# alibaba/TorchEasyRec

Measured on NVIDIA B200. Metric: samples/sec (DLRM-Criteo synth, train step fwd+bwd+optimizer), higher is better.
Workload: dtype f32

## Files before the change

### torcheasyrec_b200/csrc/tzk_gemm3x.cu

```cuda
#include <stdint.h>
#include <stdio.h>
#include <stdlib.h>

#include "tzk_umma_desc.h"
#ifdef TZK_CPU_SHIM
#include "cuda_cpu_shim.h"
#include "tcgen05_cpu_emu.h"
#else
#include <cuda.h>
#include <cuda_runtime.h>
#define TZK_DYN_SMEM(type, name) extern __shared__ __align__(1024) type name[]
#define TZK_UNPAREN(...) __VA_ARGS__
#define TZK_LAUNCH(kernel, grid, block, smem, stream, ...) TZK_UNPAREN kernel<<<grid, block, smem, stream>>>(__VA_ARGS__)
#endif

namespace {
#ifndef TZK_CPU_SHIM
#include "tzk_tcgen05_ptx.h"
#endif

constexpr int BK = 32;
constexpr int UK = 8;
constexpr int X_BYTES = BM * BK * 4;
constexpr int NUM_THREADS = 192;
template <int BN>
struct Cfg {
  static constexpr int W_BYTES = BN * BK * 4;
  static constexpr int W_PAD = (W_BYTES + 1023) / 1024 * 1024;
  static constexpr int STAGE_BYTES = 2 * X_BYTES + 2 * W_PAD;
  static constexpr int P = BN <= 64 ? 3 : 1;
  static constexpr int P_STACKED = BN <= 64 ? 2 : 1;
  static constexpr int TMEM_COLS = 512;
  static constexpr int STAGES = BN <= 64 ? 4 : 3;
};

__device__ __forceinline__ float tf32_trunc(float x) { return __uint_as_float(__float_as_uint(x) & 0xffffe000u); }

struct Params {
  const float* bias;
  float* y;
  int64_t ld_y;
  int64_t M;
  int K;
  int N;
  int relu;
};

constexpr int PF_DIST = 12;
template <int BN, bool STACK, int TW, bool RAW, bool SPLIT, bool PF>
__global__ void __launch_bounds__(64 + 32 * TW + (SPLIT ? 128 : 0), 1)
gemm3x_kernel(const __grid_constant__ CUtensorMap map_x, const __grid_constant__ CUtensorMap map_whi,
              const __grid_constant__ CUtensorMap map_wlo, Params p) {
  constexpr int W_BYTES = Cfg<BN>::W_BYTES, W_PAD = Cfg<BN>::W_PAD, STAGE_BYTES = Cfg<BN>::STAGE_BYTES;
  constexpr int TMEM_COLS = Cfg<BN>::TMEM_COLS, STAGES = Cfg<BN>::STAGES;
  constexpr int P = STACK ? Cfg<BN>::P_STACKED : Cfg<BN>::P;
  constexpr int ACC_COLS = STACK ? P * 2 * BN : (P + 1) * BN;
  static_assert(2 * ACC_COLS <= TMEM_COLS, "two tiles in flight must fit TMEM");
  static_assert(!STACK || W_PAD == W_BYTES, "stacked B needs W_hi and W_lo contiguous");
  TZK_DYN_SMEM(uint8_t, smem);
  uint8_t* stage_base = smem;
  uint64_t* bars = reinterpret_cast<uint64_t*>(smem + STAGES * STAGE_BYTES);
  uint64_t* full = bars;
  uint64_t* ready = bars + STAGES;
  uint64_t* empty = bars + 2 * STAGES;
  uint64_t* acc_full = bars + 3 * STAGES;
  uint64_t* acc_empty = bars + 3 * STAGES + 2;
  uint32_t* tmem_slot = reinterpret_cast<uint32_t*>(bars + 3 * STAGES + 4);

  const int warp = threadIdx.x >> 5, lane = threadIdx.x & 31;
  const int num_k = p.K / BK;
  const int n_used = num_k < P ? num_k : P;
  const int n_tiles = p.N / BN;
  const int64_t num_tiles = (p.M + BM - 1) / BM * n_tiles;

  if (warp == 0 && lane == 0) {
    for (int s = 0; s < STAGES; ++s) {
      mbar_init(full + s, 1);
      mbar_init(ready + s, TW);
      mbar_init(empty + s, 1);
    }
    for (int a = 0; a < 2; ++a) {
      mbar_init(acc_full + a, 1);
      mbar_init(acc_empty + a, SPLIT ? 4 : TW);
    }
    fence_mbarrier_init();
  }
  if (warp == 1) tmem_alloc(tmem_slot, TMEM_COLS);
  tc_fence_before();
  __syncthreads();
  tc_fence_after();
  const uint32_t tmem_base = *tmem_slot;

  if (warp == 0) {
    if (lane == 0) {
      int stage = 0;
      uint32_t phase = 0;
      auto load_chunk = [&](int64_t t, int kb) {
        mbar_wait(empty + stage, phase ^ 1);
        uint8_t* sb = stage_base + stage * STAGE_BYTES;
        mbar_expect_tx(full + stage, X_BYTES + 2 * W_BYTES);
        tma_load_2d(sb, &map_x, full + stage, kb * BK, (int)(t / n_tiles * BM));
        tma_load_2d(sb + 2 * X_BYTES, &map_whi, full + stage, kb * BK, (int)(t % n_tiles) * BN);
        tma_load_2d(sb + 2 * X_BYTES + W_PAD, &map_wlo, full + stage, kb * BK, (int)(t % n_tiles) * BN);
        if (++stage == STAGES) { stage = 0; phase ^= 1; }
      };
      if constexpr (PF) {
        int64_t pt = blockIdx.x;
        int pkb = 0;
        auto prefetch_next = [&] {
          if (pt < num_tiles) {
            tma_prefetch_2d(&map_x, pkb * BK, (int)(pt / n_tiles * BM));
            if (++pkb == num_k) { pkb = 0; pt += gridDim.x; }
          }
        };
        for (int i = 0; i < PF_DIST; ++i) prefetch_next();
        for (int64_t t = blockIdx.x; t < num_tiles; t += gridDim.x)
          for (int kb = 0; kb < num_k; ++kb) {
            prefetch_next();
            load_chunk(t, kb);
          }
      } else {
        for (int64_t t = blockIdx.x; t < num_tiles; t += gridDim.x)
          for (int kb = 0; kb < num_k; ++kb) load_chunk(t, kb);
      }
    }
  } else if (warp == 1) {
    int stage = 0;
    uint32_t phase = 0;
    int acc = 0;
    uint32_t acc_phase = 0;
    constexpr uint32_t idesc = make_idesc<BN>();
    constexpr uint32_t idesc2 = make_idesc<2 * BN>();
    for (int64_t t = blockIdx.x; t < num_tiles; t += gridDim.x) {
      mbar_wait_all(acc_empty + acc, acc_phase ^ 1);
      tc_fence_after();
      const uint32_t d_tmem = tmem_base + acc * ACC_COLS;
      uint32_t started = 0;
      for (int kb = 0; kb < num_k; ++kb) {
        mbar_wait_all(ready + stage, phase);
        tc_fence_after();
        if (lane == 0) {
          const uint32_t sb = smem_u32(stage_base + stage * STAGE_BYTES);
          const uint32_t a_hi = sb, a_lo = sb + X_BYTES, b_hi = sb + 2 * X_BYTES, b_lo = b_hi + W_PAD;
          const int part = kb * n_used / num_k;
#pragma unroll
          for (int k = 0; k < BK / UK; ++k) {
            const uint32_t ko = k * UK * 4;
            const uint32_t more = (started >> part) & 1u;
            if (STACK) {
              const uint32_t region = d_tmem + part * 2 * BN;
              mma_tf32(region, make_desc(a_hi + ko), make_desc(b_hi + ko), idesc2, more);
              mma_tf32(region + BN, make_desc(a_lo + ko), make_desc(b_hi + ko), idesc, 1u);
            } else {
              const uint32_t small = d_tmem + P * BN;
              mma_tf32(d_tmem + part * BN, make_desc(a_hi + ko), make_desc(b_hi + ko), idesc, more);
              mma_tf32(small, make_desc(a_lo + ko), make_desc(b_hi + ko), idesc, (started >> P) & 1u);
              mma_tf32(small, make_desc(a_hi + ko), make_desc(b_lo + ko), idesc, 1u);
            }
            started |= (1u << part) | (1u << P);
          }
          tc_commit(empty + stage);
          if (kb == num_k - 1) tc_commit(acc_full + acc);
        }
        __syncwarp();
        if (++stage == STAGES) { stage = 0; phase ^= 1; }
      }
      acc ^= 1;
      if (acc == 0) acc_phase ^= 1;
    }
  } else {
    const int tw = warp - 2;
    const int quarter = warp & 3;
    const bool do_transform = !SPLIT || tw < TW;
    const bool do_epilogue = !SPLIT || tw >= TW;
    const int part0 = SPLIT ? 0 : tw / 4, part_step = SPLIT ? 1 : TW / 4;
    int stage = 0;
    uint32_t phase = 0;
    int acc = 0;
    uint32_t acc_phase = 0;
    for (int64_t t = blockIdx.x; t < num_tiles; t += gridDim.x) {
      for (int kb = 0; do_transform && kb < num_k; ++kb) {
        mbar_wait_all(full + stage, phase);
        float4* hi = reinterpret_cast<float4*>(stage_base + stage * STAGE_BYTES);
        float4* lo = reinterpret_cast<float4*>(stage_base + stage * STAGE_BYTES + X_BYTES);
#pragma unroll
        for (int q = 0; q < X_BYTES / 16 / (TW * 32); ++q) {
          const int i = q * (TW * 32) + tw * 32 + lane;
          const float4 x = hi[i];
          float4 h, l;
          if (RAW) {
            h.x = tf32_trunc(x.x); h.y = tf32_trunc(x.y); h.z = tf32_trunc(x.z); h.w = tf32_trunc(x.w);
          } else {
            h.x = tf32_rna(x.x); h.y = tf32_rna(x.y); h.z = tf32_rna(x.z); h.w = tf32_rna(x.w);
          }
          l.x = tf32_rna(x.x - h.x); l.y = tf32_rna(x.y - h.y); l.z = tf32_rna(x.z - h.z); l.w = tf32_rna(x.w - h.w);
          if (!RAW) hi[i] = h;
          lo[i] = l;
        }
        fence_proxy_async();
        __syncwarp();
        if (lane == 0) mbar_arrive(ready + stage);
        if (++stage == STAGES) { stage = 0; phase ^= 1; }
      }
      if (!do_epilogue) continue;
      mbar_wait_all(acc_full + acc, acc_phase);
      tc_fence_after();
      const int64_t row = t / n_tiles * BM + quarter * 32 + lane;
      const int col0 = (int)(t % n_tiles) * BN;
      const uint32_t taddr = tmem_base + acc * ACC_COLS + ((uint32_t)(quarter * 32) << 16);
      float v[16];
#pragma unroll
      for (int part = part0; part < BN / 16; part += part_step) {
        float v2[16];
        if (STACK) {
          tmem_ld16(taddr + BN + part * 16, v);
          for (int q = 1; q < n_used; ++q) {
            tmem_ld16(taddr + q * 2 * BN + BN + part * 16, v2);
#pragma unroll
            for (int c = 0; c < 16; ++c) v[c] += v2[c];
          }
          for (int q = 0; q < n_used; ++q) {
            tmem_ld16(taddr + q * 2 * BN + part * 16, v2);
#pragma unroll
            for (int c = 0; c < 16; ++c) v[c] += v2[c];
          }
        } else {
          tmem_ld16(taddr + P * BN + part * 16, v);
          for (int q = 0; q < n_used; ++q) {
            tmem_ld16(taddr + q * BN + part * 16, v2);
#pragma unroll
            for (int c = 0; c < 16; ++c) v[c] += v2[c];
          }
        }
        if (row < p.M) {
          float* yr = p.y + row * p.ld_y + col0 + part * 16;
#pragma unroll
          for (int c = 0; c < 16; c += 4) {
            float4 o;
            o.x = v[c] + (p.bias ? __ldg(p.bias + col0 + part * 16 + c) : 0.f);
            o.y = v[c + 1] + (p.bias ? __ldg(p.bias + col0 + part * 16 + c + 1) : 0.f);
            o.z = v[c + 2] + (p.bias ? __ldg(p.bias + col0 + part * 16 + c + 2) : 0.f);
            o.w = v[c + 3] + (p.bias ? __ldg(p.bias + col0 + part * 16 + c + 3) : 0.f);
            if (p.relu) {
              o.x = fmaxf(o.x, 0.f); o.y = fmaxf(o.y, 0.f); o.z = fmaxf(o.z, 0.f); o.w = fmaxf(o.w, 0.f);
            }
            *reinterpret_cast<float4*>(yr + c) = o;
          }
        }
      }
      tc_fence_before();
      __syncwarp();
      if (lane == 0) mbar_arrive(acc_empty + acc);
      acc ^= 1;
      if (acc == 0) acc_phase ^= 1;
    }
  }
  tc_fence_before();
  __syncthreads();
  if (warp == 1) tmem_free(tmem_base, TMEM_COLS);
}

constexpr int WG_ROWS = 32;
constexpr int WG_BOX = WG_ROWS * 128;
constexpr int WG_A = 4 * WG_BOX, WG_B = 2 * WG_BOX;
constexpr int WG_STAGE = 2 * WG_A + 2 * WG_B;
constexpr int WG_STAGES = 4;
constexpr int WG_P = 7;

struct WgParams {
  float* partial;
  int64_t M;
  int64_t slab_rows;
  int k_tiles;
};

template <bool PF>
__global__ void __launch_bounds__(NUM_THREADS, 1)
wgrad3x_kernel(const __grid_constant__ CUtensorMap map_x, const __grid_constant__ CUtensorMap map_dz, WgParams p) {
  TZK_DYN_SMEM(uint8_t, smem);
  uint64_t* bars = reinterpret_cast<uint64_t*>(smem + WG_STAGES * WG_STAGE);
  uint64_t* full = bars;
  uint64_t* ready = bars + WG_STAGES;
  uint64_t* empty = bars + 2 * WG_STAGES;
  uint64_t* acc_full = bars + 3 * WG_STAGES;
  uint32_t* tmem_slot = reinterpret_cast<uint32_t*>(bars + 3 * WG_STAGES + 1);

  const int warp = threadIdx.x >> 5, lane = threadIdx.x & 31;
  const int jt = blockIdx.x % p.k_tiles;
  const int64_t slab = blockIdx.x / p.k_tiles;
  const int64_t row0 = slab * p.slab_rows;
  const int64_t rows = (p.M - row0 < p.slab_rows) ? p.M - row0 : p.slab_rows;
  const int num_c = (int)((rows + WG_ROWS - 1) / WG_ROWS);
  const int n_used = num_c < WG_P ? num_c : WG_P;

  if (warp == 0 && lane == 0) {
    for (int s = 0; s < WG_STAGES; ++s) {
      mbar_init(full + s, 1);
      mbar_init(ready + s, 4);
      mbar_init(empty + s, 1);
    }
    mbar_init(acc_full, 1);
    fence_mbarrier_init();
  }
  if (warp == 1) tmem_alloc(tmem_slot, 512);
  tc_fence_before();
  __syncthreads();
  tc_fence_after();
  const uint32_t tmem_base = *tmem_slot;

  if (warp == 0) {
    if (lane == 0) {
      int stage = 0;
      uint32_t phase = 0;
      if constexpr (PF) {
        for (int c = 0; c < PF_DIST && c < num_c; ++c) {
          const int r = (int)(row0 + (int64_t)c * WG_ROWS);
          for (int b = 0; b < 4; ++b) tma_prefetch_2d(&map_x, jt * 128 + b * 32, r);
          for (int b = 0; b < 2; ++b) tma_prefetch_2d(&map_dz, b * 32, r);
        }
      }
      for (int c = 0; c < num_c; ++c) {
        if constexpr (PF) {
          if (c + PF_DIST < num_c) {
            const int r = (int)(row0 + (int64_t)(c + PF_DIST) * WG_ROWS);
            for (int b = 0; b < 4; ++b) tma_prefetch_2d(&map_x, jt * 128 + b * 32, r);
            for (int b = 0; b < 2; ++b) tma_prefetch_2d(&map_dz, b * 32, r);
          }
        }
        mbar_wait(empty + stage, phase ^ 1);
        uint8_t* sb = smem + stage * WG_STAGE;
        mbar_expect_tx(full + stage, WG_A + WG_B);
        const int r = (int)(row0 + (int64_t)c * WG_ROWS);
#pragma unroll
        for (int b = 0; b < 4; ++b) tma_load_2d(sb + b * WG_BOX, &map_x, full + stage, jt * 128 + b * 32, r);
#pragma unroll
        for (int b = 0; b < 2; ++b) tma_load_2d(sb + 2 * WG_A + b * WG_BOX, &map_dz, full + stage, b * 32, r);
        if (++stage == WG_STAGES) { stage = 0; phase ^= 1; }
      }
    }
  } else if (warp == 1) {
    int stage = 0;
    uint32_t phase = 0;
    constexpr uint32_t idesc = make_idesc<64, true>();
    uint32_t started = 0;
    for (int c = 0; c < num_c; ++c) {
      mbar_wait_all(ready + stage, phase);
      tc_fence_after();
      if (lane == 0) {
        const uint32_t sb = smem_u32(smem + stage * WG_STAGE);
        const uint32_t a_hi = sb, a_lo = sb + WG_A, b_hi = sb + 2 * WG_A, b_lo = b_hi + WG_B;
        const int part = c * n_used / num_c;
        const uint32_t d_main = tmem_base + part * 64, d_small = tmem_base + WG_P * 64;
#pragma unroll
        for (int k = 0; k < WG_ROWS / UK; ++k) {
          const uint32_t ko = k * 1024;
          mma_tf32(d_main, make_desc_mn(a_hi + ko, WG_BOX, 512), make_desc_mn(b_hi + ko, WG_BOX, 512), idesc,
                   (started >> part) & 1u);
          mma_tf32(d_small, make_desc_mn(a_lo + ko, WG_BOX, 512), make_desc_mn(b_hi + ko, WG_BOX, 512), idesc,
                   (started >> WG_P) & 1u);
          mma_tf32(d_small, make_desc_mn(a_hi + ko, WG_BOX, 512), make_desc_mn(b_lo + ko, WG_BOX, 512), idesc, 1u);
          started |= (1u << part) | (1u << WG_P);
        }
        tc_commit(empty + stage);
        if (c == num_c - 1) tc_commit(acc_full);
      }
      __syncwarp();
      if (++stage == WG_STAGES) { stage = 0; phase ^= 1; }
    }
  } else {
    const int tw = warp - 2, quarter = warp & 3;
    int stage = 0;
    uint32_t phase = 0;
    for (int c = 0; c < num_c; ++c) {
      mbar_wait_all(full + stage, phase);
      uint8_t* sb = smem + stage * WG_STAGE;
#pragma unroll
      for (int q = 0; q < (WG_A + WG_B) / 16 / 128; ++q) {
        const int i = q * 128 + tw * 32 + lane;
        float4* hi = reinterpret_cast<float4*>(i < WG_A / 16 ? sb : sb + 2 * WG_A) + (i < WG_A / 16 ? i : i - WG_A / 16);
        float4* lo = reinterpret_cast<float4*>(reinterpret_cast<uint8_t*>(hi) + (i < WG_A / 16 ? WG_A : WG_B));
        const float4 x = *hi;
        float4 h, l;
        h.x = tf32_rna(x.x); h.y = tf32_rna(x.y); h.z = tf32_rna(x.z); h.w = tf32_rna(x.w);
        l.x = tf32_rna(x.x - h.x); l.y = tf32_rna(x.y - h.y); l.z = tf32_rna(x.z - h.z); l.w = tf32_rna(x.w - h.w);
        *hi = h;
        *lo = l;
      }
      fence_proxy_async();
      __syncwarp();
      if (lane == 0) mbar_arrive(ready + stage);
      if (++stage == WG_STAGES) { stage = 0; phase ^= 1; }
    }
    mbar_wait_all(acc_full, 0);
    tc_fence_after();
    const int krow = jt * 128 + quarter * 32 + lane;
    float* out = p.partial + ((int64_t)slab * p.k_tiles * 128 + krow) * 64;
    const uint32_t taddr = tmem_base + ((uint32_t)(quarter * 32) << 16);
    float v[16], v2[16];
#pragma unroll
    for (int part = 0; part < 4; ++part) {
      tmem_ld16(taddr + WG_P * 64 + part * 16, v);
      for (int q = 0; q < n_used; ++q) {
        tmem_ld16(taddr + q * 64 + part * 16, v2);
#pragma unroll
        for (int c = 0; c < 16; ++c) v[c] += v2[c];
      }
#pragma unroll
      for (int c = 0; c < 16; c += 4)
        *reinterpret_cast<float4*>(out + part * 16 + c) = make_float4(v[c], v[c + 1], v[c + 2], v[c + 3]);
    }
  }
  tc_fence_before();
  __syncthreads();
  if (warp == 1) tmem_free(tmem_base, 512);
}

__global__ void wgrad_reduce_kernel(const float* __restrict__ partial, int slabs, int k_pad, int K, float* __restrict__ dw,
                                    int64_t ld_dw) {
  const int i = blockIdx.x * blockDim.x + threadIdx.x;
  if (i >= K * 64) return;
  const int k = i >> 6, n = i & 63;
  float acc = 0.f;
  for (int s = 0; s < slabs; ++s) acc += partial[((int64_t)s * k_pad + k) * 64 + n];
  dw[(int64_t)n * ld_dw + k] = acc;
}

#ifdef TZK_CPU_SHIM
int make_map(CUtensorMap* map, const float* base, int64_t rows, int64_t cols, int64_t ld, int box_rows,
             bool atom32 = false) {
  map->base = base; map->rows = rows; map->cols = cols; map->ld = ld; map->box_rows = box_rows;
  map->atom32 = atom32;
  return 0;
}
#else
typedef CUresult (*EncodeTiled)(CUtensorMap*, CUtensorMapDataType, cuuint32_t, void*, const cuuint64_t*, const cuuint64_t*,
                                const cuuint32_t*, const cuuint32_t*, CUtensorMapInterleave, CUtensorMapSwizzle,
                                CUtensorMapL2promotion, CUtensorMapFloatOOBfill);

int make_map(CUtensorMap* map, const float* base, int64_t rows, int64_t cols, int64_t ld, int box_rows,
             bool atom32 = false) {
  static EncodeTiled encode = nullptr;
  if (!encode) {
    cudaDriverEntryPointQueryResult q;
    void* fn = nullptr;
    if (cudaGetDriverEntryPoint("cuTensorMapEncodeTiled", &fn, cudaEnableDefault, &q) != cudaSuccess || !fn) return 1;
    encode = reinterpret_cast<EncodeTiled>(fn);
  }
  cuuint64_t dims[2] = {(cuuint64_t)cols, (cuuint64_t)rows};
  cuuint64_t strides[1] = {(cuuint64_t)ld * 4};
  cuuint32_t box[2] = {(cuuint32_t)BK, (cuuint32_t)box_rows};
  cuuint32_t estr[2] = {1, 1};
  return encode(map, CU_TENSOR_MAP_DATA_TYPE_FLOAT32, 2, const_cast<float*>(base), dims, strides, box, estr,
                CU_TENSOR_MAP_INTERLEAVE_NONE, atom32 ? CU_TENSOR_MAP_SWIZZLE_128B_ATOM_32B : CU_TENSOR_MAP_SWIZZLE_128B,
                CU_TENSOR_MAP_L2_PROMOTION_L2_128B,
                CU_TENSOR_MAP_FLOAT_OOB_FILL_NONE) == CUDA_SUCCESS ? 0 : 2;
}
#endif

__global__ void split_w_kernel(const float* __restrict__ w, int64_t n, float* __restrict__ hi, float* __restrict__ lo) {
  const int64_t i = (int64_t)blockIdx.x * blockDim.x + threadIdx.x;
  if (i < n) {
    const float h = tf32_rna(w[i]);
    hi[i] = h;
    lo[i] = tf32_rna(w[i] - h);
  }
}
}

template <int BN, bool STACK, int TW, bool RAW, bool SPLIT, bool PF>
static int launch(const CUtensorMap& mx, const CUtensorMap& mh, const CUtensorMap& ml, const Params& p, cudaStream_t st) {
  const size_t smem = (size_t)Cfg<BN>::STAGES * Cfg<BN>::STAGE_BYTES + 256;
  static int sms = 0;
  if (sms == 0) {
#ifndef TZK_CPU_SHIM
    cudaFuncSetAttribute(gemm3x_kernel<BN, STACK, TW, RAW, SPLIT, PF>, cudaFuncAttributeMaxDynamicSharedMemorySize, (int)smem);
#endif
    int dev = 0, n = 148;
    cudaGetDevice(&dev);
    cudaDeviceGetAttribute(&n, cudaDevAttrMultiProcessorCount, dev);
    sms = n > 0 ? n : 148;
  }
  const int64_t tiles = (p.M + BM - 1) / BM * (p.N / BN);
  const int grid = (int)(tiles < sms ? tiles : sms);
  TZK_LAUNCH((gemm3x_kernel<BN, STACK, TW, RAW, SPLIT, PF>), grid, 64 + 32 * TW + (SPLIT ? 128 : 0), smem, st, mx, mh, ml, p);
  return cudaGetLastError() == cudaSuccess ? 0 : 3;
}

extern "C" int tzk_gemm3x(const float* x, int64_t ld_x, const float* w, int64_t ld_w, const float* bias, int64_t M,
                          int32_t N, int32_t K, int32_t relu, float* y, int64_t ld_y, float* w_hi, float* w_lo,
                          void* stream) {
  if (M <= 0 || K <= 0 || (ld_x % 4) || (ld_w % 4) || (ld_y % 4)) return 1;
  if (N != 64 && N % 112 != 0) return 1;
  cudaStream_t st = reinterpret_cast<cudaStream_t>(stream);
  const int BN = N == 64 ? 64 : 112;
  const int64_t nw = (int64_t)N * ld_w;
  TZK_LAUNCH((split_w_kernel), (unsigned)((nw + 255) / 256), 256, 0, st, w, nw, w_hi, w_lo);
  CUtensorMap mx, mh, ml;
  if (make_map(&mx, x, M, K, ld_x, BM) || make_map(&mh, w_hi, N, K, ld_w, BN) || make_map(&ml, w_lo, N, K, ld_w, BN))
    return 2;
  Params p;
  p.bias = bias; p.y = y; p.ld_y = ld_y; p.M = M; p.K = (K + BK - 1) / BK * BK; p.N = N; p.relu = relu;
  return BN == 64 ? launch<64, true, 4, false, true, false>(mx, mh, ml, p, st)
                  : launch<112, true, 4, false, true, false>(mx, mh, ml, p, st);
}

extern "C" int64_t tzk_wgrad3x_partial_floats(int32_t K, int32_t slabs) {
  return (int64_t)slabs * ((K + 127) / 128 * 128) * 64;
}
extern "C" int tzk_wgrad3x(const float* x, int64_t ld_x, const float* dz, int64_t ld_dz, int64_t M, int32_t K,
                           int32_t slabs, float* partial, float* dw, int64_t ld_dw, void* stream) {
  if (M <= 0 || K <= 0 || slabs <= 0 || (ld_x % 4) || (ld_dz % 4)) return 1;
  cudaStream_t st = reinterpret_cast<cudaStream_t>(stream);
  CUtensorMap mx, mz;
  if (make_map(&mx, x, M, K, ld_x, WG_ROWS, true) || make_map(&mz, dz, M, 64, ld_dz, WG_ROWS, true)) return 2;
  WgParams p;
  p.partial = partial;
  p.M = M;
  p.k_tiles = (K + 127) / 128;
  p.slab_rows = ((M + slabs - 1) / slabs + WG_ROWS - 1) / WG_ROWS * WG_ROWS;
  const int used = (int)((M + p.slab_rows - 1) / p.slab_rows);
  const size_t smem = (size_t)WG_STAGES * WG_STAGE + 256;
#ifndef TZK_CPU_SHIM
  static bool configured = false;
  if (!configured) {
    cudaFuncSetAttribute(wgrad3x_kernel<false>, cudaFuncAttributeMaxDynamicSharedMemorySize, (int)smem);
    configured = true;
  }
#endif
  TZK_LAUNCH((wgrad3x_kernel<false>), used * p.k_tiles, NUM_THREADS, smem, st, mx, mz, p);
  TZK_LAUNCH((wgrad_reduce_kernel), (K * 64 + 255) / 256, 256, 0, st, partial, used, p.k_tiles * 128, K, dw, ld_dw);
  return cudaGetLastError() == cudaSuccess ? 0 : 3;
}
```

### torcheasyrec_b200/csrc/tzk_tcgen05_ptx.h

```cpp

__device__ __forceinline__ uint32_t smem_u32(const void* p) { return (uint32_t)__cvta_generic_to_shared(p); }

__device__ __forceinline__ void mbar_init(uint64_t* bar, uint32_t count) {
  asm volatile("mbarrier.init.shared::cta.b64 [%0], %1;" ::"r"(smem_u32(bar)), "r"(count));
}
__device__ __forceinline__ void mbar_expect_tx(uint64_t* bar, uint32_t bytes) {
  asm volatile("mbarrier.arrive.expect_tx.shared::cta.b64 _, [%0], %1;" ::"r"(smem_u32(bar)), "r"(bytes) : "memory");
}
__device__ __forceinline__ void mbar_arrive(uint64_t* bar) {
  asm volatile("mbarrier.arrive.shared::cta.b64 _, [%0];" ::"r"(smem_u32(bar)) : "memory");
}
__device__ __forceinline__ void mbar_wait(uint64_t* bar, uint32_t parity) {
  asm volatile(
      "{\n\t.reg .pred p;\n\t"
      "WAIT_LOOP:\n\t"
      "mbarrier.try_wait.parity.shared::cta.b64 p, [%0], %1;\n\t"
      "@p bra DONE;\n\t"
      "bra WAIT_LOOP;\n\t"
      "DONE:\n\t}" ::"r"(smem_u32(bar)), "r"(parity)
      : "memory");
}

__device__ __forceinline__ void mbar_wait_all(uint64_t* bar, uint32_t parity) { mbar_wait(bar, parity); }

__device__ __forceinline__ void tma_load_2d(void* dst, const CUtensorMap* map, uint64_t* bar, int c0, int c1) {
  asm volatile(
      "cp.async.bulk.tensor.2d.shared::cluster.global.mbarrier::complete_tx::bytes [%0], [%1, {%3, %4}], [%2];"
      ::"r"(smem_u32(dst)), "l"(map), "r"(smem_u32(bar)), "r"(c0), "r"(c1)
      : "memory");
}

__device__ __forceinline__ void tma_prefetch_2d(const CUtensorMap* map, int c0, int c1) {
  asm volatile("cp.async.bulk.prefetch.tensor.2d.L2.global [%0, {%1, %2}];" ::"l"(map), "r"(c0), "r"(c1) : "memory");
}

__device__ __forceinline__ void tmem_alloc(uint32_t* dst_smem, uint32_t cols) {
  asm volatile("tcgen05.alloc.cta_group::1.sync.aligned.shared::cta.b32 [%0], %1;" ::"r"(smem_u32(dst_smem)), "r"(cols));
  asm volatile("tcgen05.relinquish_alloc_permit.cta_group::1.sync.aligned;");
}
__device__ __forceinline__ void tmem_free(uint32_t addr, uint32_t cols) {
  asm volatile("tcgen05.dealloc.cta_group::1.sync.aligned.b32 %0, %1;" ::"r"(addr), "r"(cols));
}
__device__ __forceinline__ void tc_fence_before() { asm volatile("tcgen05.fence::before_thread_sync;" ::: "memory"); }
__device__ __forceinline__ void tc_fence_after() { asm volatile("tcgen05.fence::after_thread_sync;" ::: "memory"); }
__device__ __forceinline__ void tc_commit(uint64_t* bar) {
  asm volatile("tcgen05.commit.cta_group::1.mbarrier::arrive::one.shared::cluster.b64 [%0];" ::"r"(smem_u32(bar)) : "memory");
}
__device__ __forceinline__ void mma_tf32(uint32_t tmem_d, uint64_t desc_a, uint64_t desc_b, uint32_t idesc, uint32_t accumulate) {
  asm volatile(
      "{\n\t.reg .pred p;\n\t"
      "setp.ne.b32 p, %4, 0;\n\t"
      "tcgen05.mma.cta_group::1.kind::tf32 [%0], %1, %2, %3, p;\n\t}" ::"r"(tmem_d), "l"(desc_a), "l"(desc_b), "r"(idesc),
      "r"(accumulate)
      : "memory");
}
__device__ __forceinline__ void tmem_ld16(uint32_t addr, float* v) {
  uint32_t* r = reinterpret_cast<uint32_t*>(v);
  asm volatile(
      "tcgen05.ld.sync.aligned.32x32b.x16.b32 "
      "{%0, %1, %2, %3, %4, %5, %6, %7, %8, %9, %10, %11, %12, %13, %14, %15}, [%16];"
      : "=r"(r[0]), "=r"(r[1]), "=r"(r[2]), "=r"(r[3]), "=r"(r[4]), "=r"(r[5]), "=r"(r[6]), "=r"(r[7]), "=r"(r[8]),
        "=r"(r[9]), "=r"(r[10]), "=r"(r[11]), "=r"(r[12]), "=r"(r[13]), "=r"(r[14]), "=r"(r[15])
      : "r"(addr));
  asm volatile("tcgen05.wait::ld.sync.aligned;" ::: "memory");
}

__device__ __forceinline__ float tf32_rna(float x) {
  uint32_t r;
  asm("cvt.rna.tf32.f32 %0, %1;" : "=r"(r) : "f"(x));
  return __uint_as_float(r);
}
__device__ __forceinline__ void fence_mbarrier_init() { asm volatile("fence.mbarrier_init.release.cluster;" ::: "memory"); }
__device__ __forceinline__ void fence_proxy_async() { asm volatile("fence.proxy.async.shared::cta;" ::: "memory"); }
```

Before: 70.08 million.

## Split A/B pipelines, reuse X tile across N-tiles, coalesce epilogue via smem

The GEMM kernel is restructured with separate A (activation) and B (weight) stage rings and contiguous per-CTA tile ranges. When K is small enough that all of a row-block's A chunks fit in the ring, the X tile and its split into hi/lo are loaded once and reused across consecutive N-tiles. The transform warps stop writing the rounded hi part back, since MMA consumes raw X as truncated tf32, and the epilogue is staged through shared memory so global stores are row-coalesced float4. The template variants and TMA L2 prefetch paths are removed, and the wgrad transform likewise skips rewriting the X hi half. These changes add barrier bookkeeping and rely on raw-truncation semantics for accuracy.

```diff
diff --git a/torcheasyrec_b200/csrc/tzk_gemm3x.cu b/torcheasyrec_b200/csrc/tzk_gemm3x.cu
--- a/torcheasyrec_b200/csrc/tzk_gemm3x.cu
+++ b/torcheasyrec_b200/csrc/tzk_gemm3x.cu
@@ -22,16 +22,18 @@
 constexpr int BK = 32;
 constexpr int UK = 8;
 constexpr int X_BYTES = BM * BK * 4;
+constexpr int A_STAGES = 4;
+constexpr int EPI_STRIDE = 20;
 constexpr int NUM_THREADS = 192;
 template <int BN>
 struct Cfg {
   static constexpr int W_BYTES = BN * BK * 4;
-  static constexpr int W_PAD = (W_BYTES + 1023) / 1024 * 1024;
-  static constexpr int STAGE_BYTES = 2 * X_BYTES + 2 * W_PAD;
-  static constexpr int P = BN <= 64 ? 3 : 1;
-  static constexpr int P_STACKED = BN <= 64 ? 2 : 1;
-  static constexpr int TMEM_COLS = 512;
-  static constexpr int STAGES = BN <= 64 ? 4 : 3;
+  static_assert(W_BYTES % 1024 == 0, "W_hi and W_lo must lie back to back, each 1024-B aligned");
+  static constexpr int P = BN <= 64 ? 2 : 1;
+  static constexpr int ACC_COLS = P * 2 * BN;
+  static_assert(2 * ACC_COLS <= 512, "two tiles in flight must fit TMEM");
+  static constexpr int B_STAGES = BN <= 64 ? 4 : 3;
+  static constexpr int SMEM = A_STAGES * 2 * X_BYTES + B_STAGES * 2 * W_BYTES + 4 * 32 * EPI_STRIDE * 4;
 };
 
 __device__ __forceinline__ float tf32_trunc(float x) { return __uint_as_float(__float_as_uint(x) & 0xffffe000u); }
@@ -46,46 +48,51 @@
   int relu;
 };
 
-constexpr int PF_DIST = 12;
-template <int BN, bool STACK, int TW, bool RAW, bool SPLIT, bool PF>
-__global__ void __launch_bounds__(64 + 32 * TW + (SPLIT ? 128 : 0), 1)
+template <int BN>
+__global__ void __launch_bounds__(320, 1)
 gemm3x_kernel(const __grid_constant__ CUtensorMap map_x, const __grid_constant__ CUtensorMap map_whi,
               const __grid_constant__ CUtensorMap map_wlo, Params p) {
-  constexpr int W_BYTES = Cfg<BN>::W_BYTES, W_PAD = Cfg<BN>::W_PAD, STAGE_BYTES = Cfg<BN>::STAGE_BYTES;
-  constexpr int TMEM_COLS = Cfg<BN>::TMEM_COLS, STAGES = Cfg<BN>::STAGES;
-  constexpr int P = STACK ? Cfg<BN>::P_STACKED : Cfg<BN>::P;
-  constexpr int ACC_COLS = STACK ? P * 2 * BN : (P + 1) * BN;
-  static_assert(2 * ACC_COLS <= TMEM_COLS, "two tiles in flight must fit TMEM");
-  static_assert(!STACK || W_PAD == W_BYTES, "stacked B needs W_hi and W_lo contiguous");
+  constexpr int W_BYTES = Cfg<BN>::W_BYTES, B_STAGES = Cfg<BN>::B_STAGES, P = Cfg<BN>::P, ACC_COLS = Cfg<BN>::ACC_COLS;
   TZK_DYN_SMEM(uint8_t, smem);
-  uint8_t* stage_base = smem;
-  uint64_t* bars = reinterpret_cast<uint64_t*>(smem + STAGES * STAGE_BYTES);
-  uint64_t* full = bars;
-  uint64_t* ready = bars + STAGES;
-  uint64_t* empty = bars + 2 * STAGES;
-  uint64_t* acc_full = bars + 3 * STAGES;
-  uint64_t* acc_empty = bars + 3 * STAGES + 2;
-  uint32_t* tmem_slot = reinterpret_cast<uint32_t*>(bars + 3 * STAGES + 4);
+  uint8_t* a_base = smem;
+  uint8_t* b_base = smem + A_STAGES * 2 * X_BYTES;
+  float* epi = reinterpret_cast<float*>(b_base + B_STAGES * 2 * W_BYTES);
+  uint64_t* bars = reinterpret_cast<uint64_t*>(smem + Cfg<BN>::SMEM);
+  uint64_t* a_full = bars;
+  uint64_t* a_ready = a_full + A_STAGES;
+  uint64_t* a_empty = a_ready + A_STAGES;
+  uint64_t* b_full = a_empty + A_STAGES;
+  uint64_t* b_empty = b_full + B_STAGES;
+  uint64_t* acc_full = b_empty + B_STAGES;
+  uint64_t* acc_empty = acc_full + 2;
+  uint32_t* tmem_slot = reinterpret_cast<uint32_t*>(acc_empty + 2);
 
   const int warp = threadIdx.x >> 5, lane = threadIdx.x & 31;
   const int num_k = p.K / BK;
   const int n_used = num_k < P ? num_k : P;
   const int n_tiles = p.N / BN;
   const int64_t num_tiles = (p.M + BM - 1) / BM * n_tiles;
+  const int64_t t_begin = num_tiles * blockIdx.x / gridDim.x, t_end = num_tiles * (blockIdx.x + 1) / gridDim.x;
+  const bool keep = 2 * num_k <= A_STAGES;
+  auto loads_a = [&](int64_t t) { return !keep || t == t_begin || t / n_tiles != (t - 1) / n_tiles; };
 
   if (warp == 0 && lane == 0) {
-    for (int s = 0; s < STAGES; ++s) {
-      mbar_init(full + s, 1);
-      mbar_init(ready + s, TW);
-      mbar_init(empty + s, 1);
+    for (int s = 0; s < A_STAGES; ++s) {
+      mbar_init(a_full + s, 1);
+      mbar_init(a_ready + s, 4);
+      mbar_init(a_empty + s, 1);
+    }
+    for (int s = 0; s < B_STAGES; ++s) {
+      mbar_init(b_full + s, 1);
+      mbar_init(b_empty + s, 1);
     }
     for (int a = 0; a < 2; ++a) {
       mbar_init(acc_full + a, 1);
-      mbar_init(acc_empty + a, SPLIT ? 4 : TW);
+      mbar_init(acc_empty + a, 4);
     }
     fence_mbarrier_init();
   }
-  if (warp == 1) tmem_alloc(tmem_slot, TMEM_COLS);
+  if (warp == 1) tmem_alloc(tmem_slot, 512);
   tc_fence_before();
   __syncthreads();
   tc_fence_after();
@@ -93,160 +100,137 @@
 
   if (warp == 0) {
     if (lane == 0) {
-      int stage = 0;
-      uint32_t phase = 0;
-      auto load_chunk = [&](int64_t t, int kb) {
-        mbar_wait(empty + stage, phase ^ 1);
-        uint8_t* sb = stage_base + stage * STAGE_BYTES;
-        mbar_expect_tx(full + stage, X_BYTES + 2 * W_BYTES);
-        tma_load_2d(sb, &map_x, full + stage, kb * BK, (int)(t / n_tiles * BM));
-        tma_load_2d(sb + 2 * X_BYTES, &map_whi, full + stage, kb * BK, (int)(t % n_tiles) * BN);
-        tma_load_2d(sb + 2 * X_BYTES + W_PAD, &map_wlo, full + stage, kb * BK, (int)(t % n_tiles) * BN);
-        if (++stage == STAGES) { stage = 0; phase ^= 1; }
-      };
-      if constexpr (PF) {
-        int64_t pt = blockIdx.x;
-        int pkb = 0;
-        auto prefetch_next = [&] {
-          if (pt < num_tiles) {
-            tma_prefetch_2d(&map_x, pkb * BK, (int)(pt / n_tiles * BM));
-            if (++pkb == num_k) { pkb = 0; pt += gridDim.x; }
+      int as = 0, bs = 0;
+      uint32_t aph = 0, bph = 0;
+      for (int64_t t = t_begin; t < t_end; ++t) {
+        const bool load_a = loads_a(t);
+        for (int kb = 0; kb < num_k; ++kb) {
+          if (load_a) {
+            mbar_wait(a_empty + as, aph ^ 1);
+            mbar_expect_tx(a_full + as, X_BYTES);
+            tma_load_2d(a_base + as * 2 * X_BYTES, &map_x, a_full + as, kb * BK, (int)(t / n_tiles * BM));
+            if (++as == A_STAGES) { as = 0; aph ^= 1; }
           }
-        };
-        for (int i = 0; i < PF_DIST; ++i) prefetch_next();
-        for (int64_t t = blockIdx.x; t < num_tiles; t += gridDim.x)
-          for (int kb = 0; kb < num_k; ++kb) {
-            prefetch_next();
-            load_chunk(t, kb);
-          }
-      } else {
-        for (int64_t t = blockIdx.x; t < num_tiles; t += gridDim.x)
-          for (int kb = 0; kb < num_k; ++kb) load_chunk(t, kb);
+          mbar_wait(b_empty + bs, bph ^ 1);
+          uint8_t* sb = b_base + bs * 2 * W_BYTES;
+          mbar_expect_tx(b_full + bs, 2 * W_BYTES);
+          tma_load_2d(sb, &map_whi, b_full + bs, kb * BK, (int)(t % n_tiles) * BN);
+          tma_load_2d(sb + W_BYTES, &map_wlo, b_full + bs, kb * BK, (int)(t % n_tiles) * BN);
+          if (++bs == B_STAGES) { bs = 0; bph ^= 1; }
+        }
       }
     }
   } else if (warp == 1) {
-    int stage = 0;
-    uint32_t phase = 0;
-    int acc = 0;
-    uint32_t acc_phase = 0;
+    int as = 0, bs = 0, row_as = 0, acc = 0;
+    uint32_t aph = 0, bph = 0, acc_phase = 0;
     constexpr uint32_t idesc = make_idesc<BN>();
     constexpr uint32_t idesc2 = make_idesc<2 * BN>();
-    for (int64_t t = blockIdx.x; t < num_tiles; t += gridDim.x) {
+    for (int64_t t = t_begin; t < t_end; ++t) {
+      const bool load_a = loads_a(t);
+      const bool last_use = t + 1 == t_end || loads_a(t + 1);
+      if (load_a) row_as = as;
       mbar_wait_all(acc_empty + acc, acc_phase ^ 1);
       tc_fence_after();
       const uint32_t d_tmem = tmem_base + acc * ACC_COLS;
       uint32_t started = 0;
       for (int kb = 0; kb < num_k; ++kb) {
-        mbar_wait_all(ready + stage, phase);
+        int a_slot = (row_as + kb) % A_STAGES;
+        if (load_a) {
+          a_slot = as;
+          mbar_wait_all(a_ready + as, aph);
+          if (++as == A_STAGES) { as = 0; aph ^= 1; }
+        }
+        mbar_wait_all(b_full + bs, bph);
         tc_fence_after();
         if (lane == 0) {
-          const uint32_t sb = smem_u32(stage_base + stage * STAGE_BYTES);
-          const uint32_t a_hi = sb, a_lo = sb + X_BYTES, b_hi = sb + 2 * X_BYTES, b_lo = b_hi + W_PAD;
+          const uint32_t a_hi = smem_u32(a_base + a_slot * 2 * X_BYTES), a_lo = a_hi + X_BYTES;
+          const uint32_t b_hi = smem_u32(b_base + bs * 2 * W_BYTES);
           const int part = kb * n_used / num_k;
+          const uint32_t region = d_tmem + part * 2 * BN;
 #pragma unroll
           for (int k = 0; k < BK / UK; ++k) {
             const uint32_t ko = k * UK * 4;
-            const uint32_t more = (started >> part) & 1u;
-            if (STACK) {
-              const uint32_t region = d_tmem + part * 2 * BN;
-              mma_tf32(region, make_desc(a_hi + ko), make_desc(b_hi + ko), idesc2, more);
-              mma_tf32(region + BN, make_desc(a_lo + ko), make_desc(b_hi + ko), idesc, 1u);
-            } else {
-              const uint32_t small = d_tmem + P * BN;
-              mma_tf32(d_tmem + part * BN, make_desc(a_hi + ko), make_desc(b_hi + ko), idesc, more);
-              mma_tf32(small, make_desc(a_lo + ko), make_desc(b_hi + ko), idesc, (started >> P) & 1u);
-              mma_tf32(small, make_desc(a_hi + ko), make_desc(b_lo + ko), idesc, 1u);
-            }
-            started |= (1u << part) | (1u << P);
+            mma_tf32(region, make_desc(a_hi + ko), make_desc(b_hi + ko), idesc2, ((started >> part) & 1u) | k);
+            mma_tf32(region + BN, make_desc(a_lo + ko), make_desc(b_hi + ko), idesc, 1u);
           }
-          tc_commit(empty + stage);
+          started |= 1u << part;
+          tc_commit(b_empty + bs);
+          if (last_use) tc_commit(a_empty + a_slot);
           if (kb == num_k - 1) tc_commit(acc_full + acc);
         }
         __syncwarp();
-        if (++stage == STAGES) { stage = 0; phase ^= 1; }
+        if (++bs == B_STAGES) { bs = 0; bph ^= 1; }
       }
       acc ^= 1;
       if (acc == 0) acc_phase ^= 1;
     }
+  } else if (warp < 6) {
+    const int tw = warp - 2;
+    int as = 0;
+    uint32_t aph = 0;
+    for (int64_t t = t_begin; t < t_end; ++t) {
+      if (!loads_a(t)) continue;
+      for (int kb = 0; kb < num_k; ++kb) {
+        mbar_wait_all(a_full + as, aph);
+        const float4* xs = reinterpret_cast<const float4*>(a_base + as * 2 * X_BYTES);
+        float4* lo = reinterpret_cast<float4*>(a_base + as * 2 * X_BYTES + X_BYTES);
+#pragma unroll
+        for (int q = 0; q < X_BYTES / 16 / 128; ++q) {
+          const int i = q * 128 + tw * 32 + lane;
+          const float4 x = xs[i];
+          lo[i] = make_float4(tf32_rna(x.x - tf32_trunc(x.x)), tf32_rna(x.y - tf32_trunc(x.y)),
+                              tf32_rna(x.z - tf32_trunc(x.z)), tf32_rna(x.w - tf32_trunc(x.w)));
+        }
+        fence_proxy_async();
+        __syncwarp();
+        if (lane == 0) mbar_arrive(a_ready + as);
+        if (++as == A_STAGES) { as = 0; aph ^= 1; }
+      }
+    }
   } else {
-    const int tw = warp - 2;
     const int quarter = warp & 3;
-    const bool do_transform = !SPLIT || tw < TW;
-    const bool do_epilogue = !SPLIT || tw >= TW;
-    const int part0 = SPLIT ? 0 : tw / 4, part_step = SPLIT ? 1 : TW / 4;
-    int stage = 0;
-    uint32_t phase = 0;
+    float* st = epi + (warp - 6) * 32 * EPI_STRIDE;
     int acc = 0;
     uint32_t acc_phase = 0;
-    for (int64_t t = blockIdx.x; t < num_tiles; t += gridDim.x) {
-      for (int kb = 0; do_transform && kb < num_k; ++kb) {
-        mbar_wait_all(full + stage, phase);
-        float4* hi = reinterpret_cast<float4*>(stage_base + stage * STAGE_BYTES);
-        float4* lo = reinterpret_cast<float4*>(stage_base + stage * STAGE_BYTES + X_BYTES);
-#pragma unroll
-        for (int q = 0; q < X_BYTES / 16 / (TW * 32); ++q) {
-          const int i = q * (TW * 32) + tw * 32 + lane;
-          const float4 x = hi[i];
-          float4 h, l;
-          if (RAW) {
-            h.x = tf32_trunc(x.x); h.y = tf32_trunc(x.y); h.z = tf32_trunc(x.z); h.w = tf32_trunc(x.w);
-          } else {
-            h.x = tf32_rna(x.x); h.y = tf32_rna(x.y); h.z = tf32_rna(x.z); h.w = tf32_rna(x.w);
-          }
-          l.x = tf32_rna(x.x - h.x); l.y = tf32_rna(x.y - h.y); l.z = tf32_rna(x.z - h.z); l.w = tf32_rna(x.w - h.w);
-          if (!RAW) hi[i] = h;
-          lo[i] = l;
-        }
-        fence_proxy_async();
-        __syncwarp();
-        if (lane == 0) mbar_arrive(ready + stage);
-        if (++stage == STAGES) { stage = 0; phase ^= 1; }
-      }
-      if (!do_epilogue) continue;
+    for (int64_t t = t_begin; t < t_end; ++t) {
       mbar_wait_all(acc_full + acc, acc_phase);
       tc_fence_after();
-      const int64_t row = t / n_tiles * BM + quarter * 32 + lane;
+      const int64_t row0 = t / n_tiles * BM + quarter * 32;
       const int col0 = (int)(t % n_tiles) * BN;
       const uint32_t taddr = tmem_base + acc * ACC_COLS + ((uint32_t)(quarter * 32) << 16);
-      float v[16];
-#pragma unroll
-      for (int part = part0; part < BN / 16; part += part_step) {
-        float v2[16];
-        if (STACK) {
-          tmem_ld16(taddr + BN + part * 16, v);
-          for (int q = 1; q < n_used; ++q) {
-            tmem_ld16(taddr + q * 2 * BN + BN + part * 16, v2);
-#pragma unroll
-            for (int c = 0; c < 16; ++c) v[c] += v2[c];
+#pragma unroll 1
+      for (int part = 0; part < BN / 16; ++part) {
+        float v[16], v2[16];
+        tmem_ld16(taddr + BN + part * 16, v);
+        for (int q = 1; q < n_used; ++q) {
+          tmem_ld16(taddr + q * 2 * BN + BN + part * 16, v2);
+#pragma unroll
+          for (int c = 0; c < 16; ++c) v[c] += v2[c];
+        }
+        for (int q = 0; q < n_used; ++q) {
+          tmem_ld16(taddr + q * 2 * BN + part * 16, v2);
+#pragma unroll
+          for (int c = 0; c < 16; ++c) v[c] += v2[c];
+        }
+#pragma unroll
+        for (int c = 0; c < 16; c += 4)
+          *reinterpret_cast<float4*>(st + lane * EPI_STRIDE + c) = make_float4(v[c], v[c + 1], v[c + 2], v[c + 3]);
+        __syncwarp();
+        const int c4 = (lane & 3) * 4, col = col0 + part * 16 + c4;
+        float4 bias = make_float4(0.f, 0.f, 0.f, 0.f);
+        if (p.bias) bias = make_float4(__ldg(p.bias + col), __ldg(p.bias + col + 1), __ldg(p.bias + col + 2),
+                                       __ldg(p.bias + col + 3));
+#pragma unroll
+        for (int it = 0; it < 4; ++it) {
+          const int r = it * 8 + (lane >> 2);
+          float4 o = *reinterpret_cast<const float4*>(st + r * EPI_STRIDE + c4);
+          o.x += bias.x; o.y += bias.y; o.z += bias.z; o.w += bias.w;
+          if (p.relu) {
+            o.x = fmaxf(o.x, 0.f); o.y = fmaxf(o.y, 0.f); o.z = fmaxf(o.z, 0.f); o.w = fmaxf(o.w, 0.f);
           }
-          for (int q = 0; q < n_used; ++q) {
-            tmem_ld16(taddr + q * 2 * BN + part * 16, v2);
-#pragma unroll
-            for (int c = 0; c < 16; ++c) v[c] += v2[c];
-          }
-        } else {
-          tmem_ld16(taddr + P * BN + part * 16, v);
-          for (int q = 0; q < n_used; ++q) {
-            tmem_ld16(taddr + q * BN + part * 16, v2);
-#pragma unroll
-            for (int c = 0; c < 16; ++c) v[c] += v2[c];
-          }
-        }
-        if (row < p.M) {
-          float* yr = p.y + row * p.ld_y + col0 + part * 16;
-#pragma unroll
-          for (int c = 0; c < 16; c += 4) {
-            float4 o;
-            o.x = v[c] + (p.bias ? __ldg(p.bias + col0 + part * 16 + c) : 0.f);
-            o.y = v[c + 1] + (p.bias ? __ldg(p.bias + col0 + part * 16 + c + 1) : 0.f);
-            o.z = v[c + 2] + (p.bias ? __ldg(p.bias + col0 + part * 16 + c + 2) : 0.f);
-            o.w = v[c + 3] + (p.bias ? __ldg(p.bias + col0 + part * 16 + c + 3) : 0.f);
-            if (p.relu) {
-              o.x = fmaxf(o.x, 0.f); o.y = fmaxf(o.y, 0.f); o.z = fmaxf(o.z, 0.f); o.w = fmaxf(o.w, 0.f);
-            }
-            *reinterpret_cast<float4*>(yr + c) = o;
-          }
-        }
+          if (row0 + r < p.M) *reinterpret_cast<float4*>(p.y + (row0 + r) * p.ld_y + col) = o;
+        }
+        __syncwarp();
       }
       tc_fence_before();
       __syncwarp();
@@ -257,7 +241,7 @@
   }
   tc_fence_before();
   __syncthreads();
-  if (warp == 1) tmem_free(tmem_base, TMEM_COLS);
+  if (warp == 1) tmem_free(tmem_base, 512);
 }
 
 constexpr int WG_ROWS = 32;
@@ -274,7 +258,6 @@
   int k_tiles;
 };
 
-template <bool PF>
 __global__ void __launch_bounds__(NUM_THREADS, 1)
 wgrad3x_kernel(const __grid_constant__ CUtensorMap map_x, const __grid_constant__ CUtensorMap map_dz, WgParams p) {
   TZK_DYN_SMEM(uint8_t, smem);
@@ -312,21 +295,7 @@
     if (lane == 0) {
       int stage = 0;
       uint32_t phase = 0;
-      if constexpr (PF) {
-        for (int c = 0; c < PF_DIST && c < num_c; ++c) {
-          const int r = (int)(row0 + (int64_t)c * WG_ROWS);
-          for (int b = 0; b < 4; ++b) tma_prefetch_2d(&map_x, jt * 128 + b * 32, r);
-          for (int b = 0; b < 2; ++b) tma_prefetch_2d(&map_dz, b * 32, r);
-        }
-      }
       for (int c = 0; c < num_c; ++c) {
-        if constexpr (PF) {
-          if (c + PF_DIST < num_c) {
-            const int r = (int)(row0 + (int64_t)(c + PF_DIST) * WG_ROWS);
-            for (int b = 0; b < 4; ++b) tma_prefetch_2d(&map_x, jt * 128 + b * 32, r);
-            for (int b = 0; b < 2; ++b) tma_prefetch_2d(&map_dz, b * 32, r);
-          }
-        }
         mbar_wait(empty + stage, phase ^ 1);
         uint8_t* sb = smem + stage * WG_STAGE;
         mbar_expect_tx(full + stage, WG_A + WG_B);
@@ -380,11 +349,14 @@
         float4* hi = reinterpret_cast<float4*>(i < WG_A / 16 ? sb : sb + 2 * WG_A) + (i < WG_A / 16 ? i : i - WG_A / 16);
         float4* lo = reinterpret_cast<float4*>(reinterpret_cast<uint8_t*>(hi) + (i < WG_A / 16 ? WG_A : WG_B));
         const float4 x = *hi;
-        float4 h, l;
-        h.x = tf32_rna(x.x); h.y = tf32_rna(x.y); h.z = tf32_rna(x.z); h.w = tf32_rna(x.w);
-        l.x = tf32_rna(x.x - h.x); l.y = tf32_rna(x.y - h.y); l.z = tf32_rna(x.z - h.z); l.w = tf32_rna(x.w - h.w);
-        *hi = h;
-        *lo = l;
+        float4 h;
+        if (i < WG_A / 16) {
+          h.x = tf32_trunc(x.x); h.y = tf32_trunc(x.y); h.z = tf32_trunc(x.z); h.w = tf32_trunc(x.w);
+        } else {
+          h.x = tf32_rna(x.x); h.y = tf32_rna(x.y); h.z = tf32_rna(x.z); h.w = tf32_rna(x.w);
+          *hi = h;
+        }
+        *lo = make_float4(tf32_rna(x.x - h.x), tf32_rna(x.y - h.y), tf32_rna(x.z - h.z), tf32_rna(x.w - h.w));
       }
       fence_proxy_async();
       __syncwarp();
@@ -467,13 +439,13 @@
 }
 }
 
-template <int BN, bool STACK, int TW, bool RAW, bool SPLIT, bool PF>
+template <int BN>
 static int launch(const CUtensorMap& mx, const CUtensorMap& mh, const CUtensorMap& ml, const Params& p, cudaStream_t st) {
-  const size_t smem = (size_t)Cfg<BN>::STAGES * Cfg<BN>::STAGE_BYTES + 256;
+  const size_t smem = (size_t)Cfg<BN>::SMEM + 256;
   static int sms = 0;
   if (sms == 0) {
 #ifndef TZK_CPU_SHIM
-    cudaFuncSetAttribute(gemm3x_kernel<BN, STACK, TW, RAW, SPLIT, PF>, cudaFuncAttributeMaxDynamicSharedMemorySize, (int)smem);
+    cudaFuncSetAttribute(gemm3x_kernel<BN>, cudaFuncAttributeMaxDynamicSharedMemorySize, (int)smem);
 #endif
     int dev = 0, n = 148;
     cudaGetDevice(&dev);
@@ -482,7 +454,7 @@
   }
   const int64_t tiles = (p.M + BM - 1) / BM * (p.N / BN);
   const int grid = (int)(tiles < sms ? tiles : sms);
-  TZK_LAUNCH((gemm3x_kernel<BN, STACK, TW, RAW, SPLIT, PF>), grid, 64 + 32 * TW + (SPLIT ? 128 : 0), smem, st, mx, mh, ml, p);
+  TZK_LAUNCH((gemm3x_kernel<BN>), grid, 320, smem, st, mx, mh, ml, p);
   return cudaGetLastError() == cudaSuccess ? 0 : 3;
 }
 
@@ -500,8 +472,7 @@
     return 2;
   Params p;
   p.bias = bias; p.y = y; p.ld_y = ld_y; p.M = M; p.K = (K + BK - 1) / BK * BK; p.N = N; p.relu = relu;
-  return BN == 64 ? launch<64, true, 4, false, true, false>(mx, mh, ml, p, st)
-                  : launch<112, true, 4, false, true, false>(mx, mh, ml, p, st);
+  return BN == 64 ? launch<64>(mx, mh, ml, p, st) : launch<112>(mx, mh, ml, p, st);
 }
 
 extern "C" int64_t tzk_wgrad3x_partial_floats(int32_t K, int32_t slabs) {
@@ -523,11 +494,11 @@
 #ifndef TZK_CPU_SHIM
   static bool configured = false;
   if (!configured) {
-    cudaFuncSetAttribute(wgrad3x_kernel<false>, cudaFuncAttributeMaxDynamicSharedMemorySize, (int)smem);
+    cudaFuncSetAttribute(wgrad3x_kernel, cudaFuncAttributeMaxDynamicSharedMemorySize, (int)smem);
     configured = true;
   }
 #endif
-  TZK_LAUNCH((wgrad3x_kernel<false>), used * p.k_tiles, NUM_THREADS, smem, st, mx, mz, p);
+  TZK_LAUNCH((wgrad3x_kernel), used * p.k_tiles, NUM_THREADS, smem, st, mx, mz, p);
   TZK_LAUNCH((wgrad_reduce_kernel), (K * 64 + 255) / 256, 256, 0, st, partial, used, p.k_tiles * 128, K, dw, ld_dw);
   return cudaGetLastError() == cudaSuccess ? 0 : 3;
 }
diff --git a/torcheasyrec_b200/csrc/tzk_tcgen05_ptx.h b/torcheasyrec_b200/csrc/tzk_tcgen05_ptx.h
--- a/torcheasyrec_b200/csrc/tzk_tcgen05_ptx.h
+++ b/torcheasyrec_b200/csrc/tzk_tcgen05_ptx.h
@@ -28,10 +28,6 @@
       "cp.async.bulk.tensor.2d.shared::cluster.global.mbarrier::complete_tx::bytes [%0], [%1, {%3, %4}], [%2];"
       ::"r"(smem_u32(dst)), "l"(map), "r"(smem_u32(bar)), "r"(c0), "r"(c1)
       : "memory");
-}
-
-__device__ __forceinline__ void tma_prefetch_2d(const CUtensorMap* map, int c0, int c1) {
-  asm volatile("cp.async.bulk.prefetch.tensor.2d.L2.global [%0, {%1, %2}];" ::"l"(map), "r"(c0), "r"(c1) : "memory");
 }
 
 __device__ __forceinline__ void tmem_alloc(uint32_t* dst_smem, uint32_t cols) {
```

After: 71.50 million, median of 6. +2.0%, better.
